# Viictor/vrenderer

Measured on AMD Instinct MI355X. Metric: shaded Gpixels/s at 8K terrain, higher is better.
Workload: dtype f32; 1 GPU; 7680x4320 terrain flythrough (120-frame circle r=600 y=250), heightmap 2048^2, 1 directional light; full path select+vertex+setup/bin+tile raster(PS)+deferred; heightmap=2048, nodes_last_frame=295, parallelism=screen tiles 128x128, owner=(tx+ty)%1

## Files before the change

### include/vrterrain.h

```cpp
#ifndef VRTERRAIN_H
#define VRTERRAIN_H

#include <stddef.h>
#include <stdint.h>

#ifdef __cplusplus
extern "C" {
#endif

#define VR_API __attribute__((visibility("default")))

enum {
    VR_OK = 0,
    VR_ERR_INVALID_ARGUMENT = 1,
    VR_ERR_NO_DEVICE = 2,
    VR_ERR_OUT_OF_MEMORY = 3,
    VR_ERR_TOO_MANY_INSTANCES = 4,
    VR_ERR_OVERFLOW = 5,
    VR_ERR_HIP = 6
};

#define VR_MAX_LODS 12

typedef struct vr_terrain_params {
// ... 60 lines not shown

#define VR_OWNER_TILE 128
typedef struct vr_partition {
    int32_t rank, world_size;
} vr_partition;

typedef struct vr_context  vr_context;
typedef struct vr_terrain  vr_terrain;
typedef struct vr_gbuffer  vr_gbuffer;
typedef struct vr_image    vr_image;

VR_API int  vr_context_create(int device_ordinal, vr_context** out);
VR_API void vr_context_destroy(vr_context* ctx);
VR_API int  vr_context_set_stream(vr_context* ctx, void* hip_stream);
VR_API int  vr_context_synchronize(vr_context* ctx);
enum { VR_OPT_ASYNC_GEOMETRY = 1, VR_OPT_DISPATCH_EVENTS = 2, VR_OPT_RASTER_TILE = 3, VR_OPT_PLANE_TRACKING = 4, VR_OPT_SCRATCH_WORST_CASE = 5 };
VR_API int  vr_context_set_option(vr_context* ctx, int option, int value);
VR_API const char* vr_last_error(void);
VR_API const char* vr_version(void);
VR_API uint32_t vr_build_experiments(void);

enum { VR_K_SELECT = 0, VR_K_VERTEX, VR_K_SETUP, VR_K_CLIP, VR_K_SCAN, VR_K_FILL, VR_K_RASTER,
       VR_K_DEFERRED, VR_K_DETILE, VR_K_CLEAR, VR_K_DEFERRED_TILED, VR_K_NODE_HEIGHTS,
       VR_K_TM_HISTOGRAM, VR_K_TM_EXPOSURE, VR_K_TONEMAP, VR_K_DETILE_LDR, VR_K_RASTER_DEPTH, VR_K_LIGHT_CULL, VR_K_RASTER_LIT,
       VR_K_QUERY_HEIGHTS, VR_K_QUERY_RAYS, VR_K_QUERY_PYRAMID, VR_K_COUNT };
VR_API int  vr_timing_kernel_count(void);
VR_API int  vr_timing_enable(vr_context* ctx, int enable);
VR_API int  vr_timing_collect(vr_context* ctx, float ms_sum[VR_K_COUNT], int32_t launches[VR_K_COUNT]);
VR_API const char* vr_kernel_name(int id);

VR_API int vr_view_from_camera(const float eye[3], const float target[3], const float up[3],
// ... 190 lines not shown
```

### include/vrterrain.hpp

```cpp
#pragma once

#include "vrterrain.h"

#include <array>
#include <cstdint>
#include <cstdio>
#include <functional>
#include <memory>
#include <vector>

namespace vRenderer
{
    using LogFn = std::function<void(const char*)>;
    inline LogFn& Log() { static LogFn fn = [](const char* m) { std::fprintf(stderr, "[vrterrain] %s\n", m); }; return fn; }
    inline bool Check(int rc, const char* what)
    {
        if (rc == VR_OK) return true;
        char buf[640];
        std::snprintf(buf, sizeof(buf), "%s failed (%d): %s", what, rc, vr_last_error());
        Log()(buf);
        return false;
    }

    class Device
    {
        vr_context* m_Ctx = nullptr;
    public:
        explicit Device(int ordinal = 0) { Check(vr_context_create(ordinal, &m_Ctx), "vr_context_create"); }
        ~Device() { vr_context_destroy(m_Ctx); }
        Device(const Device&) = delete;
        Device& operator=(const Device&) = delete;
        explicit operator bool() const { return m_Ctx != nullptr; }
        vr_context* Get() const { return m_Ctx; }
        void SetStream(void* hipStream) { vr_context_set_stream(m_Ctx, hipStream); }
        void WaitForIdle() { vr_context_synchronize(m_Ctx); }
    };

    struct EditorParams
    {
        bool m_RenderTerrain = true;
        bool m_Wireframe = false;
        bool m_LockView = false;
        float m_MaxHeight = 400.0f;
        uint32_t m_NumChunks = 0;
        float m_AmbientIntensity = 0.01f;
    };

    class RenderTargets
    {
// ... 223 lines not shown
```

### vrenderer_amd/capi.py

```python
import ctypes as C
import os

VR_MAX_LODS = 12
VR_OWNER_TILE = 128

VR_OK = 0
VR_ERR_INVALID_ARGUMENT = 1
VR_ERR_NO_DEVICE = 2
VR_ERR_OUT_OF_MEMORY = 3
VR_ERR_TOO_MANY_INSTANCES = 4
VR_ERR_OVERFLOW = 5
VR_ERR_HIP = 6

VR_LIGHT_DIRECTIONAL = 1
VR_LIGHT_SPOT = 2
VR_LIGHT_POINT = 3
VR_K_COUNT = 22
VR_TONEMAP_BINS = 256
VR_OPT_ASYNC_GEOMETRY = 1
VR_OPT_DISPATCH_EVENTS = 2
VR_OPT_RASTER_TILE = 3
VR_OPT_PLANE_TRACKING = 4
VR_OPT_SCRATCH_WORST_CASE = 5
VR_RAY_MISS = 0
VR_RAY_HIT = 1
VR_RAY_INVALID = 2
VR_RAY_STEP_LIMIT = 3


class TerrainParams(C.Structure):
    _fields_ = [
        ("max_instances", C.c_int32),
        ("surface_size", C.c_float),
        ("world_size", C.c_float),
        ("grid_size", C.c_int32),
        ("min_lod_distance", C.c_float),
        ("morph_start", C.c_float),
        ("location", C.c_float * 3),
# ... 262 lines not shown
```

### vrenderer_amd/csrc/vr_frame.hip

```cpp
#include "vr_internal.h"

extern "C" VR_API int vr_frame_submit(vr_terrain* t, vr_gbuffer* gb, const vr_frame_desc* f)
{
    VR_REQUIRE(t && gb && f && f->view && f->render && f->hdr_out, "NULL argument");
    VR_REQUIRE(f->num_lights >= 0 && (f->num_lights == 0 || f->lights), "lights is NULL");
    vr_context* ctx = t->ctx;
    VR_REQUIRE(gb->ctx == ctx && f->hdr_out->ctx->device == ctx->device, "G-buffer / image belong to another context");
    vr_image* hdr = f->hdr_out;
    int rc;
    int earlier = vr_terrain_render(t, f->view, f->view, gb, f->render, f->part);
    if (earlier != VR_OK && earlier != VR_ERR_TOO_MANY_INSTANCES && earlier != VR_ERR_OVERFLOW) return earlier;
    for (int k = 0; k < 2; k++)
        if (f->prepare_views[k] && (rc = vr_terrain_prepare(t, f->prepare_views[k], gb, f->render, f->part))) return rc;
    if (hdr->read_pending) { VR_HIP(hipStreamWaitEvent(ctx->stream, hdr->ev_read_done, 0)); hdr->read_pending = false; }
    if (f->tiled) rc = vr_deferred_light_tiled(ctx, f->view, gb, f->lights, f->num_lights, f->ambient_top, f->ambient_bottom, hdr, f->part);
    else if (f->shadow) rc = vr_deferred_light_shadowed(ctx, f->view, gb, f->lights, f->num_lights, f->ambient_top, f->ambient_bottom, hdr, f->part, f->shadow);
    else rc = vr_deferred_light(ctx, f->view, gb, f->lights, f->num_lights, f->ambient_top, f->ambient_bottom, hdr, f->part);
    if (rc) return rc;
    if (!f->tonemap) return earlier;

    VR_REQUIRE(f->tonemap_params && f->ldr_out, "tone-map stage: params / ldr_out missing");
    vr_context* tc = vr_tonemap_context(f->tonemap);
    VR_REQUIRE(tc->device == ctx->device, "tone mapper lives on another device");
    const bool cross = tc->stream != ctx->stream;
    if (cross) {
        hipEvent_t done = (ctx->dispatch_events && ctx->last_stop) ? ctx->last_stop : nullptr;
        if (!done) {
            if (!hdr->ev_written) VR_HIP(hipEventCreateWithFlags(&hdr->ev_written, hipEventDisableTiming));
            VR_HIP(hipEventRecord(hdr->ev_written, ctx->stream));
            done = hdr->ev_written;
        }
        VR_HIP(hipStreamWaitEvent(tc->stream, done, 0));
    }
    const int w = gb->w, h = gb->h;
    if ((rc = vr_tonemap_reset_histogram(f->tonemap))) return rc;
    if ((rc = vr_tonemap_add_frame_to_histogram(f->tonemap, f->tonemap_params, hdr, w, h, f->part))) return rc;
    if (f->nccl_comm && (rc = vr_tonemap_allreduce_histogram(f->tonemap, f->nccl_comm))) return rc;
    if ((rc = vr_tonemap_compute_exposure(f->tonemap, f->tonemap_params, f->frame_time_seconds))) return rc;
    if ((rc = vr_tonemap_render(f->tonemap, f->tonemap_params, hdr, w, h, f->ldr_out, f->ldr_capacity, f->part))) return rc;
    if (cross) {
        if (!hdr->ev_read_done) VR_HIP(hipEventCreateWithFlags(&hdr->ev_read_done, hipEventDisableTiming));
// ... 10 lines not shown
```

### vrenderer_amd/csrc/vr_host.hip

```cpp
#include "vr_internal.h"
#include "vr_experiments.h"

#include <math.h>
#include <stdarg.h>
#include <stdio.h>
#include <string.h>
#include <stdlib.h>

static thread_local char g_last_error[512] = "";
void vr_set_error(const char* fmt, ...)
{
    va_list ap; va_start(ap, fmt);
    vsnprintf(g_last_error, sizeof(g_last_error), fmt, ap);
    va_end(ap);
}
extern "C" VR_API const char* vr_last_error(void) { return g_last_error; }
extern "C" VR_API const char* vr_version(void) { return "vrterrain 0.1 (gfx950)"; }
extern "C" VR_API uint32_t vr_build_experiments(void) { return kExpMask; }

static double srgb_eotf(double c) { return c <= 0.04045 ? c / 12.92 : pow((c + 0.055) / 1.055, 2.4); }

static void timing_reset(vr_context* c);

extern "C" VR_API int vr_context_create(int device, vr_context** out)
{
    VR_REQUIRE(out != nullptr, "out is NULL");
    int n = 0;
    hipError_t e = hipGetDeviceCount(&n);
    if (e != hipSuccess || n <= 0) { vr_set_error("no HIP device available (%s)", hipGetErrorString(e)); return VR_ERR_NO_DEVICE; }
    VR_REQUIRE(device >= 0 && device < n, "device ordinal out of range");
    VR_HIP(hipSetDevice(device));
    vr_context* c = new vr_context();
    struct Guard { vr_context*& c; ~Guard() { if (c) vr_context_destroy(c); } } guard{ c };
    c->device = device;
    c->stream = nullptr;
    for (int i = 0; i < 256; i++) c->h_srgb_lut[i] = (float)srgb_eotf((double)i / 255.0);
    c->h_srgb_thr[0] = 0.0f;
    for (int k = 1; k < 256; k++) c->h_srgb_thr[k] = (float)srgb_eotf(((double)k - 0.5) / 255.0);
    VR_HIP(hipMalloc(&c->d_srgb_lut, 256 * sizeof(float)));
    VR_HIP(hipMalloc(&c->d_srgb_thr, 257 * sizeof(float)));
    VR_HIP(hipMemcpy(c->d_srgb_lut, c->h_srgb_lut, 256 * sizeof(float), hipMemcpyHostToDevice));
    VR_HIP(hipMemcpy(c->d_srgb_thr, c->h_srgb_thr, 256 * sizeof(float), hipMemcpyHostToDevice));
    { const uint32_t nan_bits = 0x7fc00000u; VR_HIP(hipMemcpy(c->d_srgb_thr + 256, &nan_bits, sizeof(nan_bits), hipMemcpyHostToDevice)); }
    {
        uint8_t tab[kEncTabSize];
        for (int b = 0; b < kEncTabSize; b++) {
            const uint32_t bits = (uint32_t)(b + kEncTabBase) << 16;
            float x; memcpy(&x, &bits, 4);
            int lo = 0, hi = 255;
            while (lo < hi) { int mid = (lo + hi + 1) >> 1; if (x >= c->h_srgb_thr[mid]) lo = mid; else hi = mid - 1; }
// ... 31 lines not shown
    for (hipEvent_t e : c->ev_pool) (void)hipEventDestroy(e);
    for (hipEvent_t e : c->ev_ring) (void)hipEventDestroy(e);
    delete c;
}

extern "C" VR_API int vr_context_set_stream(vr_context* c, void* s)
{
    VR_REQUIRE(c != nullptr, "ctx is NULL");
    c->stream = (hipStream_t)s;
    return VR_OK;
}

extern "C" VR_API int vr_context_set_option(vr_context* c, int option, int value)
{
    VR_REQUIRE(c != nullptr, "ctx is NULL");
    VR_REQUIRE(option == VR_OPT_ASYNC_GEOMETRY || option == VR_OPT_DISPATCH_EVENTS || option == VR_OPT_RASTER_TILE || option == VR_OPT_PLANE_TRACKING || option == VR_OPT_SCRATCH_WORST_CASE, "unknown option");
    if (option == VR_OPT_ASYNC_GEOMETRY) c->async_geometry = value != 0;
    else if (option == VR_OPT_PLANE_TRACKING) c->plane_tracking = value != 0;
    else if (option == VR_OPT_SCRATCH_WORST_CASE) c->scratch_worst_case = value != 0;
    else if (option == VR_OPT_RASTER_TILE) {
        VR_REQUIRE(value == 0 || value == 32 || value == 64, "VR_OPT_RASTER_TILE: 0 (by size), 32 or 64");
        c->raster_tile_force = value == 32 ? 5 : value == 64 ? 6 : 0;
    }
    else { VR_HIP(hipStreamSynchronize(c->stream)); c->dispatch_events = value != 0; c->last_stop = nullptr; }
    return VR_OK;
}

extern "C" VR_API int vr_context_synchronize(vr_context* c)
{
    VR_REQUIRE(c != nullptr, "ctx is NULL");
    VR_HIP(hipStreamSynchronize(c->stream));
    return VR_OK;
}

// ... 693 lines not shown
```

### vrenderer_amd/csrc/vr_internal.h

```cpp
#pragma once

#include <hip/hip_runtime.h>
#include <hip/hip_ext.h>
#include <stdint.h>
#include <stdlib.h>
#include <string>
#include <vector>

#include "../../include/vrterrain.h"

void vr_set_error(const char* fmt, ...);
#define VR_HIP(expr)                                                                  \
    do {                                                                              \
        hipError_t e__ = (expr);                                                      \
        if (e__ != hipSuccess) {                                                      \
            vr_set_error("%s:%d: %s -> %s", __FILE__, __LINE__, #expr, hipGetErrorString(e__)); \
            return e__ == hipErrorOutOfMemory ? VR_ERR_OUT_OF_MEMORY : VR_ERR_HIP;    \
        }                                                                             \
    } while (0)
#define VR_REQUIRE(cond, msg)                                                         \
    do { if (!(cond)) { vr_set_error("%s:%d: %s", __FILE__, __LINE__, msg); return VR_ERR_INVALID_ARGUMENT; } } while (0)

constexpr int kGrid = 32;
constexpr int kSide = kGrid + 1;
// ... 74 lines not shown
};

struct vr_context {
    int device = 0;
    hipStream_t stream = nullptr;
    hipEvent_t ev_sysfence = nullptr;
    float* d_srgb_lut = nullptr;
    float* d_srgb_thr = nullptr;
    float h_srgb_lut[256];
    float h_srgb_thr[256];
    uint8_t* d_enc_tab = nullptr;
    std::vector<PartTables*> part_tables;
    bool async_geometry = true;
    bool scratch_worst_case = false;
    bool plane_tracking = true;
    int raster_tile_force = 0;
    bool dispatch_events = true;
    std::vector<hipEvent_t> ev_ring; size_t ev_ring_pos = 0;
    hipEvent_t last_stop = nullptr;
    uint64_t ev_epoch = 1;
    DevLight* d_lights = nullptr; size_t light_capacity = 0; std::vector<DevLight> h_lights, h_lights_on_device;
    uint32_t* d_macro_scratch = nullptr; size_t macro_scratch_words = 0;
    uint32_t* d_light_lists = nullptr; size_t light_list_words = 0;
    uint32_t* d_flags = nullptr;
    int timing = 0;
    std::vector<hipEvent_t> ev_pool;
    std::vector<hipEvent_t> ev_begin, ev_end;
    std::vector<int> ev_id;
};

// ... 129 lines not shown
    hipEvent_t start_hint = nullptr;
    uint64_t start_hint_epoch = 0;
    uchar2* d_pyramid = nullptr; uint64_t pyramid_bytes = 0;
    hipEvent_t ev_pyramid = nullptr; hipStream_t pyramid_stream = nullptr;
    void* d_query_stage = nullptr; size_t query_stage_bytes = 0;
};
void vr_query_release(vr_terrain* t);

struct vr_tonemap;
vr_context* vr_tonemap_context(vr_tonemap* tm);
int vr_tex_upload_and_mip(vr_context* ctx, const uint8_t* host, int w, int h, int texel_bytes,
                          DevTex* out, uint8_t** out_mem, uint64_t* out_bytes = nullptr);
int vr_select_launch(vr_terrain* t, GeoSet& g, const vr_view* view, float max_height, hipStream_t stream);
int vr_terrain_pick_set(vr_terrain* t);
int vr_terrain_poll(vr_terrain* t, bool report);
int vr_terrain_reserve_bins(vr_terrain* t, size_t tiles);
int vr_partition_tables(vr_context* ctx, int w, int h, const vr_partition* part, const PartTables** out);
int vr_partition_slot_tables(vr_context* ctx, int w, int h, int world, const PartTables** out);

#ifndef VR_GEOMETRY_PRIO
#define VR_GEOMETRY_PRIO 3
#endif
#define VR_GEOMETRY_PRIORITY() __builtin_amdgcn_s_setprio(VR_GEOMETRY_PRIO)

__device__ __forceinline__ float vr_max(float a, float b) { return a > b ? a : b; }
__device__ __forceinline__ float vr_min(float a, float b) { return a < b ? a : b; }
__device__ __forceinline__ float vr_clampf(float x, float lo, float hi) { return __builtin_amdgcn_fmed3f(x, lo, hi); }
__device__ __forceinline__ float vr_rcp_exact(float d)
{
    const float r = __builtin_amdgcn_rcpf(d);
// ... 19 lines not shown
```

### vrenderer_amd/csrc/vr_raster.hip

```cpp
#include "vr_internal.h"
#include "vr_tex_dev.h"
#include "vr_deferred_dev.h"
#include "vr_experiments.h"
#include <type_traits>

#include <stdlib.h>
#include <string.h>

struct VertexArgs {
    float w2v[16], v2c[16];
    float cam_x, cam_z;
    float lod_ranges[VR_MAX_LODS];
    float morph_start, world_size, max_height;
    float vp_x, vp_y, vp_w, vp_h;
};

struct RasterArgs {
    int w, h;
    int vx0, vy0, vx1, vy1;
    int rtx, rty;
    int tile_shift;
    int mirrored;
    int world, rank;
    uint32_t world_magic;
// ... 962 lines not shown
#endif
constexpr int kRT = VR_RASTER_THREADS, kRW = kRT / 64;
#ifndef VR_RASTER_WAVES_PER_EU
#define VR_RASTER_WAVES_PER_EU kRW
#endif

enum { RM_GENERIC = 0, RM_FAST = 1, RM_DEPTH = 2 };
struct LitArgs {
    DeferredArgs da;
    const float* lut_g;
    uint2* hdr;
    const int32_t* tile_slot;
    int slot_base, owner_tiles_x;
};
struct LitNone { int unused; };
template <bool WIRE, int TILE, int MODE, bool RANGES = false, bool NOEMI = false, bool LIT = false>
#ifndef VR_RASTER_WAVES_32
#define VR_RASTER_WAVES_32 6
#endif
__global__ __launch_bounds__(kRT, (LIT ? 4 : TILE == 32 ? VR_RASTER_WAVES_32 : VR_RASTER_WAVES_PER_EU)) void k_raster(RasterArgs a, DevTex hm, DevTex al, const DevVert* __restrict__ verts,
                                                 const HardTriRec* __restrict__ hard_tris, const uint32_t* __restrict__ hard_first,
                                                 const uint4* __restrict__ recs, uint32_t rec_hard_base,
                                                 const uint32_t* __restrict__ tile_cursor, const uint32_t* __restrict__ tile_offset,
                                                 const TileEntry* __restrict__ entries, const int32_t* __restrict__ tile_list,
                                                 const uint32_t* __restrict__ tile_classes,
                                                 float* __restrict__ g_depth, uint32_t* __restrict__ g_diff, uint32_t* __restrict__ g_spec,
                                                 uint2* __restrict__ g_nrm, uint2* __restrict__ g_emi,
                                                 const float* __restrict__ thr_g,
                                                 const uint8_t* __restrict__ enc_g, uint32_t spec_const, uint2* __restrict__ ranges,
                                                 uint8_t* __restrict__ region,
                                                 typename std::conditional<LIT, LitArgs, LitNone>::type lit)
{
    constexpr bool TRACK = MODE == RM_FAST && TILE == 32 && !LIT && !WIRE;
    static_assert(!LIT || (MODE == RM_FAST && !RANGES), "the fused variant is the fast variant");
    static_assert((!RANGES && !NOEMI) || MODE == RM_FAST, "depth ranges and the emissive skip come with the fast variant");
    __shared__ unsigned long long vis[TILE * TILE];
    __shared__ __attribute__((aligned(4))) uint8_t enc[(kEncTabSize + 3) / 4 * 4];
    __shared__ float thr[kThrTabSize];
    __shared__ uint32_t s_qoff[kMaxLevels], s_aoff[kMaxLevels];
    __shared__ uint4 s_lv[kMaxLevels];
    __shared__ uint4 s_rec[MODE != RM_DEPTH ? 3 * (1 << kTeSlotBits) : 1];
    __shared__ float s_lut[LIT ? 256 : 1];
    const int tid = threadIdx.x, lane = tid & 63, wave = tid >> 6;
    VR_PROF_BEGIN;
    const int tile = tile_list ? tile_of_block((int)blockIdx.x, tile_list, tile_classes, a.rtx * a.rty) : (int)blockIdx.x;
    if (tile < 0 || tile >= a.rtx * a.rty) return;
    uint4 lv_r = make_uint4(0, 0, 0, 0);
    if (MODE == RM_FAST && tid < kMaxLevels) lv_r = hm.fast_lv[tid];
    uint32_t qoff_r = 0, aoff_r = 0;
    if (MODE != RM_FAST && tid < kMaxLevels) { qoff_r = hm.qoff[tid]; aoff_r = al.off[tid]; }
    constexpr int kEncWords = (kEncTabSize + 3) / 4, kEncPer = (kEncWords + kRT - 1) / kRT;
    uint32_t enc_r[kEncPer];
#pragma unroll
    for (int q = 0; q < kEncPer; q++) enc_r[q] = (!kExpNoTables && tid + q * kRT < kEncWords) ? reinterpret_cast<const uint32_t*>(enc_g)[tid + q * kRT] : 0u;
    const float thr_r = (!kExpNoTables && tid < 256) ? thr_g[tid] : 0.0f;
    float lut_r = 0.0f;
    if constexpr (LIT) lut_r = lit.lut_g[tid & 255];
    const uint32_t off = tile_offset[tile], n_all = tile_cursor[tile] - off;
    const uint32_t n = min(n_all, off < a.bin_capacity ? a.bin_capacity - off : 0u);
    const TileEntry* __restrict__ bin = entries + off;
    if constexpr (TRACK) {
        if (region != nullptr && a.assume_cleared && n_all == 0u
            && reinterpret_cast<const uint32_t*>(region)[tile] == kRegionClear * 0x01010101u) return;
    }
    const bool lds_recs = !WIRE && MODE != RM_DEPTH && n <= (uint32_t)kSparseMax;
    uint4 rec_r = make_uint4(0, 0, 0, 0);
    if (lds_recs && (uint32_t)tid < n * 3u) {
        const uint32_t ord_j = bin[(uint32_t)tid / 3u].order;
        rec_r = recs[rec_index(key_of(ord_j), hard_first, rec_hard_base) * kRecGroups + 5u + (uint32_t)tid % 3u];
    }
    const uint32_t idx0 = (uint32_t)(lane * kRW + wave);
    const int tyi = tile / a.rtx, txi = tile - tyi * a.rtx;
    const int ox = txi * TILE, oy = tyi * TILE;
    if (a.assume_cleared && ox + TILE <= a.w && oy + TILE <= a.h) {
        typedef unsigned long long u64x2 __attribute__((ext_vector_type(2)));
        const u64x2 cv = { 0x3f800000ffffffffull, 0x3f800000ffffffffull };
// ... 217 lines not shown
            const uint32_t st = region[ri];
            const int lx = tid % TILE, ly0 = (tid / TILE) * 4;
            bool c_all = true, c_none = true;
#pragma unroll
            for (int k = 0; k < 4; k++) {
                const bool on = whole || (ox + lx < a.w && oy + ly0 + k < a.h);
                const bool cov = (uint32_t)nkeys[k] != 0xffffffffu;
                c_all = c_all && (!on || cov); c_none = c_none && (!on || !cov);
            }
            const bool all_cov = __all(c_all), none_cov = __all(c_none);
            uint32_t nst;
            if (none_cov) { skip_all = a.assume_cleared ? st == kRegionClear : true; nst = a.assume_cleared ? kRegionClear : st; }
            else if (all_cov) { skip_spec = st == kRegionSpec; nst = kRegionSpec; }
            else nst = (!a.assume_cleared && st == kRegionSpec) ? kRegionSpec : 0u;
            if (nst != st && lane == 0) region[ri] = (uint8_t)nst;
        }
    }
    for (int g = skip_all ? kStrips : tid; g < kStrips; g += kRT) {
        const int lx = g % TILE, ly0 = (g / TILE) * 4;
        const int gx = ox + lx, gy0 = oy + ly0;
        const unsigned long long keys[4] = { nkeys[0], nkeys[1], nkeys[2], nkeys[3] };
        if (g + kRT < kStrips) {
            const int ny0 = ((g + kRT) / TILE) * 4;
#pragma unroll
            for (int k = 0; k < 4; k++) nkeys[k] = vis[(ny0 + k) * TILE + lx];
        } else {
#pragma unroll
            for (int k = 0; k < 4; k++) nkeys[k] = ~0ull;
        }
        const bool inside = whole || (gy0 < a.h && gx < a.w);
// ... 33 lines not shown
                    float r = vr_rcp_exact(q);
                    if (!FAST && __builtin_expect(__any(!(aq > 0x1p-60f && aq < 0x1p60f)), 0)) r = 1.0f / q;
                    p.wx = plane_at(nx0, nxx, nxy, fdx, fdy) * r;
                    p.wz = plane_at(nz0, nzx, nzy, fdx, fdy) * r;
                    p.dwxdx = __builtin_fmaf(-p.wx, qx, nxx) * r; p.dwzdx = __builtin_fmaf(-p.wz, qx, nzx) * r;
                    p.dwxdy = __builtin_fmaf(-p.wx, qy, nxy) * r; p.dwzdy = __builtin_fmaf(-p.wz, qy, nzy) * r;
                }
                VR_PROF_MARK(9);
                if (FAST) pixel_shader_fast(a, rq, rc, thr, enc, s_lv, p, dif, nn0, nn1 VR_PROF_ARG);
                else pixel_shader<false, false>(a, hm, al, rq, rc, thr, enc, s_qoff, s_aoff, p, dif, nn0, nn1);
            }
            if constexpr (LIT) {
                float lrgb[3] = { 0.0f, 0.0f, 0.0f };
                if (__any(cov)) shade_pixel<false>(lit.da, s_lut, gx, gy0 + k, __uint_as_float(dep), dif, cov ? spec_const : 0u, nn0, nn1, 0u, 0u, lrgb);
                const uint32_t o0 = vr_float_to_half(lrgb[0]) | (vr_float_to_half(lrgb[1]) << 16), o1 = vr_float_to_half(lrgb[2]);
                __builtin_amdgcn_raw_buffer_store_b32(dep, rgb, pix4, 0, aux);
                if (lit.tile_slot == nullptr) {
                    const u2 ov = { o0, o1 };
                    __builtin_nontemporal_store(ov, reinterpret_cast<u2*>(lit.hdr) + pix);
                } else {
                    const int otx = gx >> 7, oty = (gy0 + k) >> 7;
                    const int lt = lit.tile_slot[oty * lit.owner_tiles_x + otx] - lit.slot_base;
                    const size_t oi = ((size_t)lt * VR_OWNER_TILE + (size_t)((gy0 + k) & 127)) * VR_OWNER_TILE + (size_t)(gx & 127);
                    uint16_t* dst = reinterpret_cast<uint16_t*>(lit.hdr) + oi * 3;
                    dst[0] = (uint16_t)o0; dst[1] = (uint16_t)(o0 >> 16); dst[2] = (uint16_t)o1;
                }
                continue;
            }
            if (kExpNoStore) {
                if (a.w < 0) __builtin_amdgcn_raw_buffer_store_b32(dep ^ dif ^ nn0 ^ nn1, rgb, pix4, 0, aux);
                continue;
            }
            if (gb_small) {
                __builtin_amdgcn_raw_buffer_store_b32(dep, rgb, pix4, 0, aux);
                if (!depth_only) {
                    const uint32_t pix8 = pix4 + pix4;
                    __builtin_amdgcn_raw_buffer_store_b32(dif, rgb, pix4, o_diff, aux);
                    if (!skip_spec) __builtin_amdgcn_raw_buffer_store_b32(cov ? spec_const : 0u, rgb, pix4, o_spec, aux);
                    const u2 nv = { nn0, nn1 }, zv = { 0u, 0u };
                    __builtin_amdgcn_raw_buffer_store_b64(nv, rgb, pix8, o_nrm, aux);
                    if (!NOEMI && !kExpNoEmissive) __builtin_amdgcn_raw_buffer_store_b64(zv, rgb, pix8, o_emi, aux);
                }
// ... 174 lines not shown
        if (p.prepared && prepared_matches(p, view, rp, gb->w, gb->h, a)) return VR_OK;
    GeoSet& g = t->sets[vr_terrain_pick_set(t)];
    g.prepared = false;
    if (t->raster_begin_recorded && (t->start_hint_epoch == 0 || t->start_hint_epoch == t->ctx->ev_epoch))
        VR_HIP(hipStreamWaitEvent(t->geo_streams[t->geo_turn & 1u], t->start_hint, 0));
    if ((rc = launch_geometry(t, g, nullptr, view, rp, a, pt))) return rc;
    bool other_prepared = false;
    for (const GeoSet& p : t->sets) other_prepared |= (&p != &g) && p.prepared;
    if (other_prepared) g.main_waited = false;
    else { VR_HIP(hipStreamWaitEvent(t->ctx->stream, g.ev_geo_done, 0)); g.main_waited = true; g.main_wait_stream = t->ctx->stream; }
    g.prepared = true; g.prep_view = *view; g.prep_rp = *rp; g.prep_w = gb->w; g.prep_h = gb->h; g.prep_rank = a.rank; g.prep_world = a.world; g.prep_tile_shift = a.tile_shift;
    g.prep_serial = ++t->prep_counter;
    return VR_OK;
}

struct LitRequest { const vr_light* lights; int32_t num_lights; const float* amb_top; const float* amb_bottom; vr_image* hdr; };
static int terrain_render_impl(vr_terrain* t, const vr_view* view, vr_gbuffer* gb, const vr_render_params* rp, const vr_partition* part,
                               const LitRequest* lit_req, bool* lit_done, int* earlier_out);

extern "C" VR_API int vr_terrain_render(vr_terrain* t, const vr_view* view, const vr_view* view_prev, vr_gbuffer* gb,
                                         const vr_render_params* rp, const vr_partition* part)
{
    (void)view_prev;
    int earlier = VR_OK;
    const int rc = terrain_render_impl(t, view, gb, rp, part, nullptr, nullptr, &earlier);
    return rc ? rc : earlier;
}

extern "C" VR_API int vr_terrain_render_lit(vr_terrain* t, const vr_view* view, vr_gbuffer* gb, const vr_render_params* rp,
                                             const vr_partition* part, const vr_light* lights, int32_t num_lights,
                                             const float ambient_top[3], const float ambient_bottom[3], vr_image* hdr_out)
{
    VR_REQUIRE(t && view && gb && rp && hdr_out && ambient_top && ambient_bottom, "NULL argument");
    VR_REQUIRE(rp->assume_cleared && !rp->depth_only && !rp->wireframe && !rp->depth_ranges,
               "vr_terrain_render_lit draws into a cleared target (assume_cleared = 1), shaded fill mode, no depth ranges");
    VR_REQUIRE(num_lights >= 0 && num_lights <= kMaxLights && (num_lights == 0 || lights), "at most 16 lights (terrain_cb.h:15)");
    const LitRequest req = { lights, num_lights, ambient_top, ambient_bottom, hdr_out };
    bool fused = false;
    int earlier = VR_OK;
    int rc = terrain_render_impl(t, view, gb, rp, part, &req, &fused, &earlier);
    if (rc) return rc;
    if (!fused && (rc = vr_deferred_light(t->ctx, view, gb, lights, num_lights, ambient_top, ambient_bottom, hdr_out, part))) return rc;
    return earlier;
}

static int terrain_render_impl(vr_terrain* t, const vr_view* view, vr_gbuffer* gb, const vr_render_params* rp, const vr_partition* part,
                               const LitRequest* lit_req, bool* lit_done, int* earlier_out)
{
    int rc = check_render_inputs(t, view, gb, rp);
    if (rc) return rc;
    vr_context* ctx = t->ctx;
    VR_HIP(hipSetDevice(ctx->device));
    hipStream_t s = ctx->stream;
    const int earlier = vr_terrain_poll(t, true);
    if (earlier && earlier != VR_ERR_OVERFLOW && earlier != VR_ERR_TOO_MANY_INSTANCES) return earlier;
    RasterArgs a;
    if ((rc = make_raster_args(t, view, rp, gb->w, gb->h, part, a))) return rc;
    if ((rc = vr_terrain_reserve_bins(t, (size_t)a.rtx * a.rty / (size_t)(a.world > 1 ? a.world : 1)))) return rc;
    a.bin_capacity = (uint32_t)t->bin_capacity;
    const PartTables* pt = nullptr;
    if (a.world > 1 && (rc = vr_partition_tables(ctx, gb->w, gb->h, part, &pt))) return rc;
    if (gb->clear_pending) {
        if (a.world <= 1 && !a.depth_only && lit_req == nullptr) { a.assume_cleared = 1; gb->clear_pending = false; }
        else if ((rc = vr_gbuffer_materialise(gb, s))) return rc;
    }

    int gi = -1;
    if (!rp->lock_view)
        for (int i = 0; i < kGeoSets; i++)
            if (i != t->cur && t->sets[i].prepared && prepared_matches(t->sets[i], view, rp, gb->w, gb->h, a)) { gi = i; break; }
    const bool use_prepared = gi >= 0;
    if (!use_prepared) gi = vr_terrain_pick_set(t);
    GeoSet& g = t->sets[gi];
    GeoSet& last = t->sets[t->cur];
    g.prepared = false;
    if (!use_prepared) {
        GeoSet* sel = (rp->lock_view && last.have_selection) ? &last : nullptr;
        if ((rc = launch_geometry(t, g, sel, view, rp, a, pt))) return rc;
    }
    t->cur = gi;
    if (!(use_prepared && g.main_waited && g.main_wait_stream == s)) VR_HIP(hipStreamWaitEvent(s, g.ev_geo_done, 0));
    g.main_waited = false;
    const uint32_t spec_const = vr_specular_constant(ctx);
    const int grid = pt ? pt->num_raster_tiles : a.rtx * a.rty;
    if (ctx->dispatch_events && ctx->last_stop) { t->start_hint = ctx->last_stop; t->start_hint_epoch = ctx->ev_epoch; t->raster_begin_recorded = true; }
    else { VR_HIP(hipEventRecord(t->ev_raster_begin, s)); t->start_hint = t->ev_raster_begin; t->start_hint_epoch = 0; t->raster_begin_recorded = true; }
    hipEvent_t pass_stop = nullptr;
    if (grid > 0) {
        VrKernelScope ks(ctx, rp->depth_only ? VR_K_RASTER_DEPTH : VR_K_RASTER, s, true);
        const int32_t* tiles = g.d_tile_order;
        const bool same = t->height.w0 == t->albedo.w0 && t->height.h0 == t->albedo.h0 && t->height.levels == t->albedo.levels;
        const uint64_t span = (uint64_t)((const char*)(gb->emissive + (size_t)gb->w * gb->h) - (const char*)gb->depth);
        const bool one_rsrc = (const char*)gb->depth < (const char*)gb->diffuse && (const char*)gb->depth < (const char*)gb->specular
                           && (const char*)gb->depth < (const char*)gb->normals && (const char*)gb->depth < (const char*)gb->emissive && span < (1ull << 32);
        const bool fast = same && a.ws_pow2 && one_rsrc && !a.wireframe && !a.depth_only;
        const bool depth = a.depth_only && !a.wireframe;
        const bool ranges = rp->depth_ranges && fast && a.assume_cleared && !gb->escaped;
        if (ranges) {
            if ((rc = vr_gbuffer_ranges_prepare(gb, s))) return rc;
            gb->ranges_state = vr_gbuffer::RANGES_VALID; gb->ranges_rank = a.rank; gb->ranges_world = a.world;
        } else vr_gbuffer_touch(gb);
        const bool noemi = fast && ctx->plane_tracking && gb->emissive_zero && !gb->escaped;
        auto kern = a.tile_shift == 5 ? pick_raster<32>(a.wireframe != 0, fast, depth, ranges, noemi) : pick_raster<64>(a.wireframe != 0, fast, depth, ranges, noemi);
        LitArgs la;
        bool fuse = false;
        if (lit_req && fast && !ranges) {
            bool extra = false;
            memset(&la, 0, sizeof(la));
            if ((rc = vr_deferred_make_args(view, gb->w, gb->h, lit_req->lights, lit_req->num_lights, lit_req->amb_top, lit_req->amb_bottom, &la.da, &extra))) return rc;
            VR_REQUIRE(view->viewport_w == gb->w && view->viewport_h == gb->h && view->viewport_x == 0 && view->viewport_y == 0,
                       "view viewport must cover the G-buffer");
            fuse = !extra && gb->w % 4 == 0;
            if (fuse) {
                la.lut_g = ctx->d_srgb_lut; la.hdr = (uint2*)lit_req->hdr->data;
                if (pt) {
                    VR_REQUIRE((size_t)pt->max_owned * VR_OWNER_TILE * VR_OWNER_TILE * 6 <= lit_req->hdr->capacity_bytes, "hdr_out is smaller than vr_partition_packed_bytes()");
                    la.tile_slot = pt->d_tile_slot; la.slot_base = pt->rank * pt->max_owned; la.owner_tiles_x = (gb->w + VR_OWNER_TILE - 1) / VR_OWNER_TILE;
                    la.da.tiles_x = la.owner_tiles_x;
                } else VR_REQUIRE((size_t)gb->w * gb->h * 8 <= lit_req->hdr->capacity_bytes, "hdr_out is smaller than the frame");
            }
        }
        if (lit_done) *lit_done = fuse;
        uint8_t* region = nullptr;
        if (fast && !fuse && a.tile_shift == 5 && ctx->plane_tracking && !gb->escaped) { if ((rc = vr_gbuffer_region_prepare(gb, s, &region))) return rc; }
        else gb->region_fill = 0;
#define VR_RASTER_ARGS a, t->height, t->albedo, g.d_verts, g.d_hard_tris, g.d_hard_first, \
                           (const uint4*)g.d_recs, (uint32_t)t->cap_instances * (uint32_t)kTrisPerInst, g.d_tile_cursor, g.d_tile_offset, g.d_bin_entries, tiles, g.d_counters + C_CLASS0, \
                           gb->depth, gb->diffuse, gb->specular, gb->normals, gb->emissive, ctx->d_srgb_thr, ctx->d_enc_tab, spec_const, ranges ? gb->d_ranges : (uint2*)nullptr, region
        if (fuse) {
            ks.id = VR_K_RASTER_LIT;
            if (a.tile_shift == 5) VR_LAUNCH_TIMED(ks, (k_raster<false, 32, RM_FAST, false, true, true>), dim3(grid), dim3(kRT), s, VR_RASTER_ARGS, la);
            else VR_LAUNCH_TIMED(ks, (k_raster<false, 64, RM_FAST, false, true, true>), dim3(grid), dim3(kRT), s, VR_RASTER_ARGS, la);
        } else
        VR_LAUNCH_TIMED(ks, kern, dim3(grid), dim3(kRT), s, VR_RASTER_ARGS, LitNone());
#undef VR_RASTER_ARGS
        if (ctx->dispatch_events && ks.e0 && ks.e1) pass_stop = ks.e1;
        if (!fuse && !noemi && !a.depth_only && a.assume_cleared && a.world <= 1) gb->emissive_zero = true;
    }
    if (pass_stop) { g.raster_done = pass_stop; g.raster_done_epoch = ctx->ev_epoch; }
    else { VR_HIP(hipEventRecord(g.ev_raster_done, s)); g.raster_done = g.ev_raster_done; g.raster_done_epoch = 0; }
    g.raster_recorded = true;
    for (GeoSet& p : t->sets)
        if (&p != &g && p.prepared && !(p.main_waited && p.main_wait_stream == s) && p.geo_recorded) { VR_HIP(hipStreamWaitEvent(s, p.ev_geo_done, 0)); p.main_waited = true; p.main_wait_stream = s; }
    VR_HIP(hipGetLastError());
    if (earlier_out) *earlier_out = earlier;
    return VR_OK;
}

extern "C" VR_API int vr_debug_tile_order(vr_terrain* t, int32_t* out_tiles, uint32_t* out_bin_lengths, int32_t capacity, int32_t* out_count)
{
    VR_REQUIRE(t && out_tiles && out_bin_lengths && out_count && capacity >= 0, "bad arguments");
// ... 28 lines not shown
```

### vrenderer_amd/passes.py

```python
import ctypes as C

import numpy as np

from . import capi
from .capi import (GBufferDesc, Instance, Light, Partition, RenderParams, TerrainParams, View, check)


def _vp(a):
    return a.ctypes.data_as(C.c_void_p)


def _f3(v):
    return (C.c_float * 3)(*[float(x) for x in v])


RAY_DTYPE = np.dtype([("origin", np.float32, 3), ("t_max", np.float32), ("dir", np.float32, 3), ("reserved", np.uint32)])
RAY_HIT_DTYPE = np.dtype([("t", np.float32), ("position", np.float32, 3), ("normal", np.float32, 3), ("status", np.uint32)])
assert RAY_DTYPE.itemsize == C.sizeof(capi.Ray) == 32 and RAY_HIT_DTYPE.itemsize == C.sizeof(capi.RayHit) == 32


def pixel_ray(view, px, py):
    r = capi.Ray()
    check(capi.load_library().vr_view_pixel_ray(C.byref(view), px, py, C.byref(r)), "vr_view_pixel_ray")
    return r
# ... 13 lines not shown

    def synchronize(self):
        check(self.lib.vr_context_synchronize(self.handle), "vr_context_synchronize")

    def set_async_geometry(self, enable):
        check(self.lib.vr_context_set_option(self.handle, capi.VR_OPT_ASYNC_GEOMETRY, int(enable)), "vr_context_set_option")

    def set_raster_tile(self, edge):
        check(self.lib.vr_context_set_option(self.handle, capi.VR_OPT_RASTER_TILE, int(edge)), "vr_context_set_option")

    def set_plane_tracking(self, enable):
        check(self.lib.vr_context_set_option(self.handle, capi.VR_OPT_PLANE_TRACKING, int(enable)), "vr_context_set_option")

    def set_scratch_worst_case(self, enable):
        check(self.lib.vr_context_set_option(self.handle, capi.VR_OPT_SCRATCH_WORST_CASE, int(enable)), "vr_context_set_option")

    def set_dispatch_events(self, enable):
        check(self.lib.vr_context_set_option(self.handle, capi.VR_OPT_DISPATCH_EVENTS, int(enable)), "vr_context_set_option")

    def timing_enable(self, enable=True):
        check(self.lib.vr_timing_enable(self.handle, int(enable)), "vr_timing_enable")

    def timing_collect(self):
        ms = (C.c_float * capi.VR_K_COUNT)()
        n = (C.c_int32 * capi.VR_K_COUNT)()
        check(self.lib.vr_timing_collect(self.handle, ms, n), "vr_timing_collect")
        return {self.lib.vr_kernel_name(i).decode(): (float(ms[i]), int(n[i])) for i in range(capi.VR_K_COUNT) if n[i]}

    def close(self):
        if getattr(self, "handle", None):
# ... 565 lines not shown
```

Baseline: 78.68 Gpixels/s.

## Fuse deferred lighting into tile raster while keeping the G-buffer in frame submit

Adds a frame-fusion path, on by default, in which vr_frame_submit calls a new render_keep entry point. It runs a LIT+KEEP raster kernel that shades each pixel and writes HDR output directly, still writing the G-buffer but skipping the separate deferred-lighting pass over the full 8K frame. Empty tiles skipped by plane tracking now write zero HDR instead of returning early. The aim is to remove a whole-screen G-buffer reread and a kernel launch, at the cost of higher register pressure in the raster kernel (launch bounds set to 5 waves) and extra writes for empty tiles.

```diff
diff --git a/include/vrterrain.h b/include/vrterrain.h
--- a/include/vrterrain.h
+++ b/include/vrterrain.h
@@ -98,7 +98,8 @@
 VR_API void vr_context_destroy(vr_context* ctx);
 VR_API int  vr_context_set_stream(vr_context* ctx, void* hip_stream);
 VR_API int  vr_context_synchronize(vr_context* ctx);
-enum { VR_OPT_ASYNC_GEOMETRY = 1, VR_OPT_DISPATCH_EVENTS = 2, VR_OPT_RASTER_TILE = 3, VR_OPT_PLANE_TRACKING = 4, VR_OPT_SCRATCH_WORST_CASE = 5 };
+enum { VR_OPT_ASYNC_GEOMETRY = 1, VR_OPT_DISPATCH_EVENTS = 2, VR_OPT_RASTER_TILE = 3, VR_OPT_PLANE_TRACKING = 4, VR_OPT_SCRATCH_WORST_CASE = 5,
+       VR_OPT_FRAME_FUSION = 6 };
 VR_API int  vr_context_set_option(vr_context* ctx, int option, int value);
 VR_API const char* vr_last_error(void);
 VR_API const char* vr_version(void);
diff --git a/include/vrterrain.hpp b/include/vrterrain.hpp
--- a/include/vrterrain.hpp
+++ b/include/vrterrain.hpp
@@ -33,6 +33,8 @@
         explicit operator bool() const { return m_Ctx != nullptr; }
         vr_context* Get() const { return m_Ctx; }
         void SetStream(void* hipStream) { vr_context_set_stream(m_Ctx, hipStream); }
+        void SetOption(int option, int value) { Check(vr_context_set_option(m_Ctx, option, value), "vr_context_set_option"); }
+        void SetFrameFusion(bool enable) { SetOption(VR_OPT_FRAME_FUSION, enable ? 1 : 0); }
         void WaitForIdle() { vr_context_synchronize(m_Ctx); }
     };
 
diff --git a/vrenderer_amd/capi.py b/vrenderer_amd/capi.py
--- a/vrenderer_amd/capi.py
+++ b/vrenderer_amd/capi.py
@@ -22,6 +22,7 @@
 VR_OPT_RASTER_TILE = 3
 VR_OPT_PLANE_TRACKING = 4
 VR_OPT_SCRATCH_WORST_CASE = 5
+VR_OPT_FRAME_FUSION = 6
 VR_RAY_MISS = 0
 VR_RAY_HIT = 1
 VR_RAY_INVALID = 2
diff --git a/vrenderer_amd/csrc/vr_frame.hip b/vrenderer_amd/csrc/vr_frame.hip
--- a/vrenderer_amd/csrc/vr_frame.hip
+++ b/vrenderer_amd/csrc/vr_frame.hip
@@ -8,14 +8,22 @@
     VR_REQUIRE(gb->ctx == ctx && f->hdr_out->ctx->device == ctx->device, "G-buffer / image belong to another context");
     vr_image* hdr = f->hdr_out;
     int rc;
-    int earlier = vr_terrain_render(t, f->view, f->view, gb, f->render, f->part);
+    bool fused = false;
+    hipEvent_t fused_stop = nullptr;
+    int earlier;
+    if (ctx->frame_fusion && !f->tiled && !f->shadow && !f->part)
+        earlier = vr_terrain_render_keep(t, f->view, gb, f->render, f->lights, f->num_lights, f->ambient_top, f->ambient_bottom, hdr, &fused, &fused_stop);
+    else earlier = vr_terrain_render(t, f->view, f->view, gb, f->render, f->part);
     if (earlier != VR_OK && earlier != VR_ERR_TOO_MANY_INSTANCES && earlier != VR_ERR_OVERFLOW) return earlier;
     for (int k = 0; k < 2; k++)
         if (f->prepare_views[k] && (rc = vr_terrain_prepare(t, f->prepare_views[k], gb, f->render, f->part))) return rc;
+    if (fused) rc = VR_OK;
+    else {
     if (hdr->read_pending) { VR_HIP(hipStreamWaitEvent(ctx->stream, hdr->ev_read_done, 0)); hdr->read_pending = false; }
     if (f->tiled) rc = vr_deferred_light_tiled(ctx, f->view, gb, f->lights, f->num_lights, f->ambient_top, f->ambient_bottom, hdr, f->part);
     else if (f->shadow) rc = vr_deferred_light_shadowed(ctx, f->view, gb, f->lights, f->num_lights, f->ambient_top, f->ambient_bottom, hdr, f->part, f->shadow);
     else rc = vr_deferred_light(ctx, f->view, gb, f->lights, f->num_lights, f->ambient_top, f->ambient_bottom, hdr, f->part);
+    }
     if (rc) return rc;
     if (!f->tonemap) return earlier;
 
@@ -24,7 +32,7 @@
     VR_REQUIRE(tc->device == ctx->device, "tone mapper lives on another device");
     const bool cross = tc->stream != ctx->stream;
     if (cross) {
-        hipEvent_t done = (ctx->dispatch_events && ctx->last_stop) ? ctx->last_stop : nullptr;
+        hipEvent_t done = fused ? fused_stop : (ctx->dispatch_events && ctx->last_stop) ? ctx->last_stop : nullptr;
         if (!done) {
             if (!hdr->ev_written) VR_HIP(hipEventCreateWithFlags(&hdr->ev_written, hipEventDisableTiming));
             VR_HIP(hipEventRecord(hdr->ev_written, ctx->stream));
diff --git a/vrenderer_amd/csrc/vr_host.hip b/vrenderer_amd/csrc/vr_host.hip
--- a/vrenderer_amd/csrc/vr_host.hip
+++ b/vrenderer_amd/csrc/vr_host.hip
@@ -34,6 +34,7 @@
     struct Guard { vr_context*& c; ~Guard() { if (c) vr_context_destroy(c); } } guard{ c };
     c->device = device;
     c->stream = nullptr;
+    if (const char* e = getenv("VR_FRAME_FUSION")) c->frame_fusion = atoi(e) != 0;
     for (int i = 0; i < 256; i++) c->h_srgb_lut[i] = (float)srgb_eotf((double)i / 255.0);
     c->h_srgb_thr[0] = 0.0f;
     for (int k = 1; k < 256; k++) c->h_srgb_thr[k] = (float)srgb_eotf(((double)k - 0.5) / 255.0);
@@ -95,10 +96,11 @@
 extern "C" VR_API int vr_context_set_option(vr_context* c, int option, int value)
 {
     VR_REQUIRE(c != nullptr, "ctx is NULL");
-    VR_REQUIRE(option == VR_OPT_ASYNC_GEOMETRY || option == VR_OPT_DISPATCH_EVENTS || option == VR_OPT_RASTER_TILE || option == VR_OPT_PLANE_TRACKING || option == VR_OPT_SCRATCH_WORST_CASE, "unknown option");
+    VR_REQUIRE(option == VR_OPT_ASYNC_GEOMETRY || option == VR_OPT_DISPATCH_EVENTS || option == VR_OPT_RASTER_TILE || option == VR_OPT_PLANE_TRACKING || option == VR_OPT_SCRATCH_WORST_CASE || option == VR_OPT_FRAME_FUSION, "unknown option");
     if (option == VR_OPT_ASYNC_GEOMETRY) c->async_geometry = value != 0;
     else if (option == VR_OPT_PLANE_TRACKING) c->plane_tracking = value != 0;
     else if (option == VR_OPT_SCRATCH_WORST_CASE) c->scratch_worst_case = value != 0;
+    else if (option == VR_OPT_FRAME_FUSION) c->frame_fusion = value != 0;
     else if (option == VR_OPT_RASTER_TILE) {
         VR_REQUIRE(value == 0 || value == 32 || value == 64, "VR_OPT_RASTER_TILE: 0 (by size), 32 or 64");
         c->raster_tile_force = value == 32 ? 5 : value == 64 ? 6 : 0;
diff --git a/vrenderer_amd/csrc/vr_internal.h b/vrenderer_amd/csrc/vr_internal.h
--- a/vrenderer_amd/csrc/vr_internal.h
+++ b/vrenderer_amd/csrc/vr_internal.h
@@ -112,6 +112,7 @@
     bool async_geometry = true;
     bool scratch_worst_case = false;
     bool plane_tracking = true;
+    bool frame_fusion = true;
     int raster_tile_force = 0;
     bool dispatch_events = true;
     std::vector<hipEvent_t> ev_ring; size_t ev_ring_pos = 0;
@@ -271,6 +272,9 @@
 int vr_select_launch(vr_terrain* t, GeoSet& g, const vr_view* view, float max_height, hipStream_t stream);
 int vr_terrain_pick_set(vr_terrain* t);
 int vr_terrain_poll(vr_terrain* t, bool report);
+int vr_terrain_render_keep(vr_terrain* t, const vr_view* view, vr_gbuffer* gb, const vr_render_params* rp, const vr_light* lights,
+                           int32_t num_lights, const float ambient_top[3], const float ambient_bottom[3], vr_image* hdr_out,
+                           bool* fused, hipEvent_t* fused_stop);
 int vr_terrain_reserve_bins(vr_terrain* t, size_t tiles);
 int vr_partition_tables(vr_context* ctx, int w, int h, const vr_partition* part, const PartTables** out);
 int vr_partition_slot_tables(vr_context* ctx, int w, int h, int world, const PartTables** out);
diff --git a/vrenderer_amd/csrc/vr_raster.hip b/vrenderer_amd/csrc/vr_raster.hip
--- a/vrenderer_amd/csrc/vr_raster.hip
+++ b/vrenderer_amd/csrc/vr_raster.hip
@@ -1000,11 +1000,14 @@
     int slot_base, owner_tiles_x;
 };
 struct LitNone { int unused; };
-template <bool WIRE, int TILE, int MODE, bool RANGES = false, bool NOEMI = false, bool LIT = false>
+#ifndef VR_RASTER_WAVES_KEEP
+#define VR_RASTER_WAVES_KEEP 5
+#endif
+template <bool WIRE, int TILE, int MODE, bool RANGES = false, bool NOEMI = false, bool LIT = false, bool KEEP = false>
 #ifndef VR_RASTER_WAVES_32
 #define VR_RASTER_WAVES_32 6
 #endif
-__global__ __launch_bounds__(kRT, (LIT ? 4 : TILE == 32 ? VR_RASTER_WAVES_32 : VR_RASTER_WAVES_PER_EU)) void k_raster(RasterArgs a, DevTex hm, DevTex al, const DevVert* __restrict__ verts,
+__global__ __launch_bounds__(kRT, (KEEP ? VR_RASTER_WAVES_KEEP : LIT ? 4 : TILE == 32 ? VR_RASTER_WAVES_32 : VR_RASTER_WAVES_PER_EU)) void k_raster(RasterArgs a, DevTex hm, DevTex al, const DevVert* __restrict__ verts,
                                                  const HardTriRec* __restrict__ hard_tris, const uint32_t* __restrict__ hard_first,
                                                  const uint4* __restrict__ recs, uint32_t rec_hard_base,
                                                  const uint32_t* __restrict__ tile_cursor, const uint32_t* __restrict__ tile_offset,
@@ -1017,7 +1020,8 @@
                                                  uint8_t* __restrict__ region,
                                                  typename std::conditional<LIT, LitArgs, LitNone>::type lit)
 {
-    constexpr bool TRACK = MODE == RM_FAST && TILE == 32 && !LIT && !WIRE;
+    constexpr bool TRACK = MODE == RM_FAST && TILE == 32 && (!LIT || KEEP) && !WIRE;
+    static_assert(!KEEP || (LIT && NOEMI && TILE == 32), "the G-buffer-keeping flavour: fused, 32-pixel tiles, emissive plane known zero");
     static_assert(!LIT || (MODE == RM_FAST && !RANGES), "the fused variant is the fast variant");
     static_assert((!RANGES && !NOEMI) || MODE == RM_FAST, "depth ranges and the emissive skip come with the fast variant");
     __shared__ unsigned long long vis[TILE * TILE];
@@ -1045,7 +1049,7 @@
     const uint32_t off = tile_offset[tile], n_all = tile_cursor[tile] - off;
     const uint32_t n = min(n_all, off < a.bin_capacity ? a.bin_capacity - off : 0u);
     const TileEntry* __restrict__ bin = entries + off;
-    if constexpr (TRACK) {
+    if constexpr (TRACK && !KEEP) {
         if (region != nullptr && a.assume_cleared && n_all == 0u
             && reinterpret_cast<const uint32_t*>(region)[tile] == kRegionClear * 0x01010101u) return;
     }
@@ -1293,6 +1297,21 @@
             else if (all_cov) { skip_spec = st == kRegionSpec; nst = kRegionSpec; }
             else nst = (!a.assume_cleared && st == kRegionSpec) ? kRegionSpec : 0u;
             if (nst != st && lane == 0) region[ri] = (uint8_t)nst;
+        }
+    }
+    if constexpr (KEEP) {
+        if (skip_all) {
+            for (int g = tid; g < kStrips; g += kRT) {
+                const int gx = ox + g % TILE, gy0 = oy + (g / TILE) * 4;
+                if (!whole && gx >= a.w) continue;
+#pragma unroll
+                for (int k = 0; k < 4; k++) {
+                    if (!whole && gy0 + k >= a.h) break;
+                    const u2 zv = { 0u, 0u };
+                    __builtin_nontemporal_store(zv, reinterpret_cast<u2*>(lit.hdr) + ((uint32_t)__umul24(gy0 + k, a.w) + (uint32_t)gx));
+                }
+            }
+            return;
         }
     }
     for (int g = skip_all ? kStrips : tid; g < kStrips; g += kRT) {
@@ -1356,8 +1375,8 @@
                 float lrgb[3] = { 0.0f, 0.0f, 0.0f };
                 if (__any(cov)) shade_pixel<false>(lit.da, s_lut, gx, gy0 + k, __uint_as_float(dep), dif, cov ? spec_const : 0u, nn0, nn1, 0u, 0u, lrgb);
                 const uint32_t o0 = vr_float_to_half(lrgb[0]) | (vr_float_to_half(lrgb[1]) << 16), o1 = vr_float_to_half(lrgb[2]);
-                __builtin_amdgcn_raw_buffer_store_b32(dep, rgb, pix4, 0, aux);
-                if (lit.tile_slot == nullptr) {
+                if constexpr (!KEEP) __builtin_amdgcn_raw_buffer_store_b32(dep, rgb, pix4, 0, aux);
+                if (KEEP || lit.tile_slot == nullptr) {
                     const u2 ov = { o0, o1 };
                     __builtin_nontemporal_store(ov, reinterpret_cast<u2*>(lit.hdr) + pix);
                 } else {
@@ -1367,7 +1386,7 @@
                     uint16_t* dst = reinterpret_cast<uint16_t*>(lit.hdr) + oi * 3;
                     dst[0] = (uint16_t)o0; dst[1] = (uint16_t)(o0 >> 16); dst[2] = (uint16_t)o1;
                 }
-                continue;
+                if constexpr (!KEEP) continue;
             }
             if (kExpNoStore) {
                 if (a.w < 0) __builtin_amdgcn_raw_buffer_store_b32(dep ^ dif ^ nn0 ^ nn1, rgb, pix4, 0, aux);
@@ -1572,7 +1591,8 @@
     return VR_OK;
 }
 
-struct LitRequest { const vr_light* lights; int32_t num_lights; const float* amb_top; const float* amb_bottom; vr_image* hdr; };
+struct LitRequest { const vr_light* lights; int32_t num_lights; const float* amb_top; const float* amb_bottom; vr_image* hdr;
+                    bool keep; hipEvent_t* stop_out; };
 static int terrain_render_impl(vr_terrain* t, const vr_view* view, vr_gbuffer* gb, const vr_render_params* rp, const vr_partition* part,
                                const LitRequest* lit_req, bool* lit_done, int* earlier_out);
 
@@ -1593,13 +1613,24 @@
     VR_REQUIRE(rp->assume_cleared && !rp->depth_only && !rp->wireframe && !rp->depth_ranges,
                "vr_terrain_render_lit draws into a cleared target (assume_cleared = 1), shaded fill mode, no depth ranges");
     VR_REQUIRE(num_lights >= 0 && num_lights <= kMaxLights && (num_lights == 0 || lights), "at most 16 lights (terrain_cb.h:15)");
-    const LitRequest req = { lights, num_lights, ambient_top, ambient_bottom, hdr_out };
+    const LitRequest req = { lights, num_lights, ambient_top, ambient_bottom, hdr_out, false, nullptr };
     bool fused = false;
     int earlier = VR_OK;
     int rc = terrain_render_impl(t, view, gb, rp, part, &req, &fused, &earlier);
     if (rc) return rc;
     if (!fused && (rc = vr_deferred_light(t->ctx, view, gb, lights, num_lights, ambient_top, ambient_bottom, hdr_out, part))) return rc;
     return earlier;
+}
+
+int vr_terrain_render_keep(vr_terrain* t, const vr_view* view, vr_gbuffer* gb, const vr_render_params* rp, const vr_light* lights,
+                           int32_t num_lights, const float ambient_top[3], const float ambient_bottom[3], vr_image* hdr_out,
+                           bool* fused, hipEvent_t* fused_stop)
+{
+    const LitRequest req = { lights, num_lights, ambient_top, ambient_bottom, hdr_out, true, fused_stop };
+    int earlier = VR_OK;
+    *fused = false; *fused_stop = nullptr;
+    const int rc = terrain_render_impl(t, view, gb, rp, nullptr, &req, fused, &earlier);
+    return rc ? rc : earlier;
 }
 
 static int terrain_render_impl(vr_terrain* t, const vr_view* view, vr_gbuffer* gb, const vr_render_params* rp, const vr_partition* part,
@@ -1618,8 +1649,31 @@
     a.bin_capacity = (uint32_t)t->bin_capacity;
     const PartTables* pt = nullptr;
     if (a.world > 1 && (rc = vr_partition_tables(ctx, gb->w, gb->h, part, &pt))) return rc;
+    const bool same = t->height.w0 == t->albedo.w0 && t->height.h0 == t->albedo.h0 && t->height.levels == t->albedo.levels;
+    const uint64_t span = (uint64_t)((const char*)(gb->emissive + (size_t)gb->w * gb->h) - (const char*)gb->depth);
+    const bool one_rsrc = (const char*)gb->depth < (const char*)gb->diffuse && (const char*)gb->depth < (const char*)gb->specular
+                       && (const char*)gb->depth < (const char*)gb->normals && (const char*)gb->depth < (const char*)gb->emissive && span < (1ull << 32);
+    const bool fast = same && a.ws_pow2 && one_rsrc && !a.wireframe && !a.depth_only;
+    LitArgs la;
+    bool keep = false;
+    if (lit_req && lit_req->keep) {
+        const bool cleared = rp->assume_cleared || gb->clear_pending;
+        keep = part == nullptr && fast && a.tile_shift == 5 && cleared && !rp->depth_ranges
+            && ctx->plane_tracking && gb->emissive_zero && !gb->escaped
+            && view->viewport_w == gb->w && view->viewport_h == gb->h && view->viewport_x == 0 && view->viewport_y == 0 && gb->w % 4 == 0
+            && lit_req->amb_top && lit_req->amb_bottom && lit_req->hdr && lit_req->hdr->data
+            && lit_req->num_lights >= 0 && lit_req->num_lights <= kMaxLights && (lit_req->num_lights == 0 || lit_req->lights)
+            && (size_t)gb->w * gb->h * 8 <= lit_req->hdr->capacity_bytes && lit_req->hdr->ctx->device == ctx->device;
+        if (keep) {
+            bool extra = false;
+            memset(&la, 0, sizeof(la));
+            keep = vr_deferred_make_args(view, gb->w, gb->h, lit_req->lights, lit_req->num_lights, lit_req->amb_top, lit_req->amb_bottom, &la.da, &extra) == VR_OK
+                && !extra;
+        }
+        if (!keep) lit_req = nullptr;
+    }
     if (gb->clear_pending) {
-        if (a.world <= 1 && !a.depth_only && lit_req == nullptr) { a.assume_cleared = 1; gb->clear_pending = false; }
+        if (a.world <= 1 && !a.depth_only && (lit_req == nullptr || keep)) { a.assume_cleared = 1; gb->clear_pending = false; }
         else if ((rc = vr_gbuffer_materialise(gb, s))) return rc;
     }
 
@@ -1647,11 +1701,6 @@
     if (grid > 0) {
         VrKernelScope ks(ctx, rp->depth_only ? VR_K_RASTER_DEPTH : VR_K_RASTER, s, true);
         const int32_t* tiles = g.d_tile_order;
-        const bool same = t->height.w0 == t->albedo.w0 && t->height.h0 == t->albedo.h0 && t->height.levels == t->albedo.levels;
-        const uint64_t span = (uint64_t)((const char*)(gb->emissive + (size_t)gb->w * gb->h) - (const char*)gb->depth);
-        const bool one_rsrc = (const char*)gb->depth < (const char*)gb->diffuse && (const char*)gb->depth < (const char*)gb->specular
-                           && (const char*)gb->depth < (const char*)gb->normals && (const char*)gb->depth < (const char*)gb->emissive && span < (1ull << 32);
-        const bool fast = same && a.ws_pow2 && one_rsrc && !a.wireframe && !a.depth_only;
         const bool depth = a.depth_only && !a.wireframe;
         const bool ranges = rp->depth_ranges && fast && a.assume_cleared && !gb->escaped;
         if (ranges) {
@@ -1660,9 +1709,11 @@
         } else vr_gbuffer_touch(gb);
         const bool noemi = fast && ctx->plane_tracking && gb->emissive_zero && !gb->escaped;
         auto kern = a.tile_shift == 5 ? pick_raster<32>(a.wireframe != 0, fast, depth, ranges, noemi) : pick_raster<64>(a.wireframe != 0, fast, depth, ranges, noemi);
-        LitArgs la;
-        bool fuse = false;
-        if (lit_req && fast && !ranges) {
+        bool fuse = keep;
+        if (keep) {
+            la.lut_g = ctx->d_srgb_lut; la.hdr = (uint2*)lit_req->hdr->data;
+            if (lit_req->hdr->read_pending) { VR_HIP(hipStreamWaitEvent(s, lit_req->hdr->ev_read_done, 0)); lit_req->hdr->read_pending = false; }
+        } else if (lit_req && fast && !ranges) {
             bool extra = false;
             memset(&la, 0, sizeof(la));
             if ((rc = vr_deferred_make_args(view, gb->w, gb->h, lit_req->lights, lit_req->num_lights, lit_req->amb_top, lit_req->amb_bottom, &la.da, &extra))) return rc;
@@ -1680,19 +1731,21 @@
         }
         if (lit_done) *lit_done = fuse;
         uint8_t* region = nullptr;
-        if (fast && !fuse && a.tile_shift == 5 && ctx->plane_tracking && !gb->escaped) { if ((rc = vr_gbuffer_region_prepare(gb, s, &region))) return rc; }
+        if (fast && (!fuse || keep) && a.tile_shift == 5 && ctx->plane_tracking && !gb->escaped) { if ((rc = vr_gbuffer_region_prepare(gb, s, &region))) return rc; }
         else gb->region_fill = 0;
 #define VR_RASTER_ARGS a, t->height, t->albedo, g.d_verts, g.d_hard_tris, g.d_hard_first, \
                            (const uint4*)g.d_recs, (uint32_t)t->cap_instances * (uint32_t)kTrisPerInst, g.d_tile_cursor, g.d_tile_offset, g.d_bin_entries, tiles, g.d_counters + C_CLASS0, \
                            gb->depth, gb->diffuse, gb->specular, gb->normals, gb->emissive, ctx->d_srgb_thr, ctx->d_enc_tab, spec_const, ranges ? gb->d_ranges : (uint2*)nullptr, region
         if (fuse) {
             ks.id = VR_K_RASTER_LIT;
-            if (a.tile_shift == 5) VR_LAUNCH_TIMED(ks, (k_raster<false, 32, RM_FAST, false, true, true>), dim3(grid), dim3(kRT), s, VR_RASTER_ARGS, la);
+            if (keep) VR_LAUNCH_TIMED(ks, (k_raster<false, 32, RM_FAST, false, true, true, true>), dim3(grid), dim3(kRT), s, VR_RASTER_ARGS, la);
+            else if (a.tile_shift == 5) VR_LAUNCH_TIMED(ks, (k_raster<false, 32, RM_FAST, false, true, true>), dim3(grid), dim3(kRT), s, VR_RASTER_ARGS, la);
             else VR_LAUNCH_TIMED(ks, (k_raster<false, 64, RM_FAST, false, true, true>), dim3(grid), dim3(kRT), s, VR_RASTER_ARGS, la);
         } else
         VR_LAUNCH_TIMED(ks, kern, dim3(grid), dim3(kRT), s, VR_RASTER_ARGS, LitNone());
 #undef VR_RASTER_ARGS
         if (ctx->dispatch_events && ks.e0 && ks.e1) pass_stop = ks.e1;
+        if (keep && lit_req->stop_out) *lit_req->stop_out = pass_stop;
         if (!fuse && !noemi && !a.depth_only && a.assume_cleared && a.world <= 1) gb->emissive_zero = true;
     }
     if (pass_stop) { g.raster_done = pass_stop; g.raster_done_epoch = ctx->ev_epoch; }
diff --git a/vrenderer_amd/passes.py b/vrenderer_amd/passes.py
--- a/vrenderer_amd/passes.py
+++ b/vrenderer_amd/passes.py
@@ -51,6 +51,9 @@
 
     def set_scratch_worst_case(self, enable):
         check(self.lib.vr_context_set_option(self.handle, capi.VR_OPT_SCRATCH_WORST_CASE, int(enable)), "vr_context_set_option")
+
+    def set_frame_fusion(self, enable):
+        check(self.lib.vr_context_set_option(self.handle, capi.VR_OPT_FRAME_FUSION, int(enable)), "vr_context_set_option")
 
     def set_dispatch_events(self, enable):
         check(self.lib.vr_context_set_option(self.handle, capi.VR_OPT_DISPATCH_EVENTS, int(enable)), "vr_context_set_option")
```

Result: faster. 85.77 Gpixels/s, median of 6 (+9.0%).
